# fpthink/EPC-Net

Measured on AMD Instinct MI355X. Metric: point-clouds/sec (4096 pts) descriptor extraction, higher is better.
Workload: dtype f16x3; 1 GPU; epc-net inference, batch 64x4096x3 fp32 per GPU, NetVLAD K=64, 256-D output (BASELINE.json configs[1]); num_points=4096, precision=EPC_PRECISION_F32 (include/epcnet.h), weights=seeded random init of the architecture (no checkpoint payloads exist), parallelism=independent clouds sharded over 1 GPU(s), no data-path collective

## Files before the change

### epc-net_amd/csrc/knn.hip

```cpp
#include "train_common.h"
#include <stdlib.h>

#define KNN_THREADS 1024
#define KNN_TILE 1024
#define KNN_CT 32
#define KNN_WAVES (KNN_THREADS / 64)
#define KNN_LDS_MAX_N 8192

__device__ __forceinline__ int fkey(float v) {
    const int b = __float_as_int(v);
    return b ^ ((b >> 31) & 0x7fffffff);
}
__device__ __forceinline__ float fkey_inv(int k) { return __int_as_float(k ^ ((k >> 31) & 0x7fffffff)); }

template <int KSEL>
__device__ __forceinline__ void topk_insert(float (&top)[KSEL], float v) {
#pragma unroll
    for (int s = 0; s < KSEL; ++s) {
        const float hi = fmaxf(top[s], v);
        v = fminf(top[s], v);
        top[s] = hi;
    }
}

__device__ __forceinline__ void topk_insert_key(int (&top)[20], int v) {
    int t;
    asm(
        "v_min_i32 %[t], %[k0], %[v]\n\tv_max_i32 %[k0], %[k0], %[v]\n\t"
        "v_min_i32 %[v], %[k1], %[t]\n\tv_max_i32 %[k1], %[k1], %[t]\n\t"
        "v_min_i32 %[t], %[k2], %[v]\n\tv_max_i32 %[k2], %[k2], %[v]\n\t"
        "v_min_i32 %[v], %[k3], %[t]\n\tv_max_i32 %[k3], %[k3], %[t]\n\t"
        "v_min_i32 %[t], %[k4], %[v]\n\tv_max_i32 %[k4], %[k4], %[v]\n\t"
        "v_min_i32 %[v], %[k5], %[t]\n\tv_max_i32 %[k5], %[k5], %[t]\n\t"
        "v_min_i32 %[t], %[k6], %[v]\n\tv_max_i32 %[k6], %[k6], %[v]\n\t"
        "v_min_i32 %[v], %[k7], %[t]\n\tv_max_i32 %[k7], %[k7], %[t]\n\t"
        "v_min_i32 %[t], %[k8], %[v]\n\tv_max_i32 %[k8], %[k8], %[v]\n\t"
        "v_min_i32 %[v], %[k9], %[t]\n\tv_max_i32 %[k9], %[k9], %[t]\n\t"
        "v_min_i32 %[t], %[k10], %[v]\n\tv_max_i32 %[k10], %[k10], %[v]\n\t"
        "v_min_i32 %[v], %[k11], %[t]\n\tv_max_i32 %[k11], %[k11], %[t]\n\t"
        "v_min_i32 %[t], %[k12], %[v]\n\tv_max_i32 %[k12], %[k12], %[v]\n\t"
        "v_min_i32 %[v], %[k13], %[t]\n\tv_max_i32 %[k13], %[k13], %[t]\n\t"
        "v_min_i32 %[t], %[k14], %[v]\n\tv_max_i32 %[k14], %[k14], %[v]\n\t"
        "v_min_i32 %[v], %[k15], %[t]\n\tv_max_i32 %[k15], %[k15], %[t]\n\t"
        "v_min_i32 %[t], %[k16], %[v]\n\tv_max_i32 %[k16], %[k16], %[v]\n\t"
        "v_min_i32 %[v], %[k17], %[t]\n\tv_max_i32 %[k17], %[k17], %[t]\n\t"
        "v_min_i32 %[t], %[k18], %[v]\n\tv_max_i32 %[k18], %[k18], %[v]\n\t"
        "v_min_i32 %[v], %[k19], %[t]\n\tv_max_i32 %[k19], %[k19], %[t]\n\t"
        : [v] "+v"(v), [t] "=&v"(t), [k0] "+v"(top[0]), [k1] "+v"(top[1]), [k2] "+v"(top[2]), [k3] "+v"(top[3]), [k4] "+v"(top[4]), [k5] "+v"(top[5]), [k6] "+v"(top[6]), [k7] "+v"(top[7]), [k8] "+v"(top[8]), [k9] "+v"(top[9]), [k10] "+v"(top[10]), [k11] "+v"(top[11]), [k12] "+v"(top[12]), [k13] "+v"(top[13]), [k14] "+v"(top[14]), [k15] "+v"(top[15]), [k16] "+v"(top[16]), [k17] "+v"(top[17]), [k18] "+v"(top[18]), [k19] "+v"(top[19]));
}

__device__ __forceinline__ void topk_insert_dist(float (&top)[20], float v) {
    asm(
        "v_med3_f32 %[k19], %[k18], %[k19], %[v]\n\t"
        "v_med3_f32 %[k18], %[k17], %[k18], %[v]\n\t"
        "v_med3_f32 %[k17], %[k16], %[k17], %[v]\n\t"
        "v_med3_f32 %[k16], %[k15], %[k16], %[v]\n\t"
        "v_med3_f32 %[k15], %[k14], %[k15], %[v]\n\t"
        "v_med3_f32 %[k14], %[k13], %[k14], %[v]\n\t"
        "v_med3_f32 %[k13], %[k12], %[k13], %[v]\n\t"
        "v_med3_f32 %[k12], %[k11], %[k12], %[v]\n\t"
        "v_med3_f32 %[k11], %[k10], %[k11], %[v]\n\t"
        "v_med3_f32 %[k10], %[k9], %[k10], %[v]\n\t"
        "v_med3_f32 %[k9], %[k8], %[k9], %[v]\n\t"
        "v_med3_f32 %[k8], %[k7], %[k8], %[v]\n\t"
        "v_med3_f32 %[k7], %[k6], %[k7], %[v]\n\t"
        "v_med3_f32 %[k6], %[k5], %[k6], %[v]\n\t"
        "v_med3_f32 %[k5], %[k4], %[k5], %[v]\n\t"
        "v_med3_f32 %[k4], %[k3], %[k4], %[v]\n\t"
        "v_med3_f32 %[k3], %[k2], %[k3], %[v]\n\t"
        "v_med3_f32 %[k2], %[k1], %[k2], %[v]\n\t"
        "v_med3_f32 %[k1], %[k0], %[k1], %[v]\n\t"
        "v_min_f32 %[k0], %[k0], %[v]\n\t"
        : [k0] "+v"(top[0]), [k1] "+v"(top[1]), [k2] "+v"(top[2]), [k3] "+v"(top[3]), [k4] "+v"(top[4]), [k5] "+v"(top[5]), [k6] "+v"(top[6]), [k7] "+v"(top[7]), [k8] "+v"(top[8]), [k9] "+v"(top[9]), [k10] "+v"(top[10]), [k11] "+v"(top[11]), [k12] "+v"(top[12]), [k13] "+v"(top[13]), [k14] "+v"(top[14]), [k15] "+v"(top[15]), [k16] "+v"(top[16]), [k17] "+v"(top[17]), [k18] "+v"(top[18]), [k19] "+v"(top[19])
        : [v] "v"(v));
}

__device__ __forceinline__ bool wave_any(bool p) { return __builtin_amdgcn_ballot_w64(p) != 0ull; }

#define KNN_BATCH 8
#define KNN_MASK_WORDS (KNN_LDS_MAX_N / KNN_BATCH / 32)
static_assert(32 % (KNN_CT / KNN_BATCH) == 0, "a tile's batch bits must not straddle a mask word");

template <int KSEL, bool CONV1, int BATCH>
__global__ __launch_bounds__(KNN_THREADS, BATCH == 4 ? 8 : 1) void knn_topk_culled_kernel(const float* __restrict__ xyz, int n, int cap,
                                                                      int32_t* __restrict__ idx,
                                                                      int32_t* __restrict__ cnt,
                                                                      float* __restrict__ kth_out,
                                                                      const float* __restrict__ conv1_pack,
                                                                      float* __restrict__ x32,
                                                                      unsigned short* __restrict__ x16, int idx_u16,
                                                                      int32_t* __restrict__ status) {
    extern __shared__ __attribute__((aligned(16))) float4 cand[];
    const int ntiles = (n + KNN_CT - 1) / KNN_CT;
    const int npad = ntiles * KNN_CT;
    float4* bb = cand + npad;
    float* s_margin = reinterpret_cast<float*>(bb + 2 * ntiles);
    constexpr int BPT = KNN_CT / BATCH;
    constexpr int MASKW = KNN_LDS_MAX_N / BATCH / 32;
    static_assert(32 % BPT == 0, "a tile's batch bits must not straddle a mask word");
    unsigned int* hitmask = reinterpret_cast<unsigned int*>(s_margin + 4) + (threadIdx.x >> 6) * MASKW;
    const int cloud = blockIdx.y;
    const int tid = threadIdx.x, lane = tid & 63, wave = __builtin_amdgcn_readfirstlane(tid >> 6);
    const float* pc = xyz + (size_t)cloud * n * 3;

    bool bad = false;
    for (int j = tid; j < npad; j += KNN_THREADS) {
        float4 v = make_float4(0.f, 0.f, 0.f, INFINITY);
        if (j < n) {
            v.x = pc[3 * j + 0];
            v.y = pc[3 * j + 1];
            v.z = pc[3 * j + 2];
            v.w = sq3(v.x, v.y, v.z);
            bad |= !(v.w <= 3.4028234664e38f);
        }
        cand[j] = v;
    }
    if (status && blockIdx.x == 0 && wave_any(bad) && lane == 0) atomicOr(status + cloud, EPC_STATUS_NONFINITE_INPUT);
    __syncthreads();
    if constexpr (CONV1) {
        const int q = tid & 15;
        const float4 w0 = *reinterpret_cast<const float4*>(conv1_pack + 4 * q);
        const float4 w1 = *reinterpret_cast<const float4*>(conv1_pack + 64 + 4 * q);
        const float4 w2 = *reinterpret_cast<const float4*>(conv1_pack + 128 + 4 * q);
        const float4 b = *reinterpret_cast<const float4*>(conv1_pack + 192 + 4 * q);
        const int p0 = blockIdx.x * KNN_THREADS;
        const int np = min(KNN_THREADS, n - p0);
        bool ovf = false;
        for (int t = tid; t < np * 16; t += KNN_THREADS) {
            const int g = p0 + (t >> 4);
            const float4 pt = cand[g];
            const float4 y = conv1_quad(pt.x, pt.y, pt.z, w0, w1, w2, b);
            const size_t row = (size_t)cloud * n + g;
            if (x32) *reinterpret_cast<float4*>(x32 + row * 64 + 4 * q) = y;
            if (x16) {
                reinterpret_cast<uint2*>(x16)[row * 16 + q] = pack_half4(y);
                ovf |= fmaxf(fmaxf(y.x, y.y), fmaxf(y.z, y.w)) > 65504.0f;
            }
        }
        if (status && x16 && wave_any(ovf) && lane == 0) atomicOr(status + cloud, EPC_STATUS_FP16_RANGE);
    }
    for (int t = wave * (64 / KNN_CT) + lane / KNN_CT; t < ntiles; t += KNN_WAVES * (64 / KNN_CT)) {
        const float4 v = cand[t * KNN_CT + (lane % KNN_CT)];
        const bool ok = v.w != INFINITY;
        float lx = ok ? v.x : INFINITY, ly = ok ? v.y : INFINITY, lz = ok ? v.z : INFINITY;
        float hx = ok ? v.x : -INFINITY, hy = ok ? v.y : -INFINITY, hz = ok ? v.z : -INFINITY;
#pragma unroll
        for (int off = KNN_CT / 2; off >= 1; off >>= 1) {
            lx = fminf(lx, __shfl_xor(lx, off));
            ly = fminf(ly, __shfl_xor(ly, off));
            lz = fminf(lz, __shfl_xor(lz, off));
            hx = fmaxf(hx, __shfl_xor(hx, off));
            hy = fmaxf(hy, __shfl_xor(hy, off));
            hz = fmaxf(hz, __shfl_xor(hz, off));
        }
        if ((lane % KNN_CT) == 0) {
            bb[2 * t] = make_float4(lx, ly, lz, 0.f);
            bb[2 * t + 1] = make_float4(hx, hy, hz, 0.f);
        }
    }
    __syncthreads();
    if (wave == 0) {
        float m = 0.f;
        for (int t = lane; t < ntiles; t += 64) {
            const float4 lo = bb[2 * t], hi = bb[2 * t + 1];
            const float ax = fmaxf(fabsf(lo.x), fabsf(hi.x)), ay = fmaxf(fabsf(lo.y), fabsf(hi.y)),
                        az = fmaxf(fabsf(lo.z), fabsf(hi.z));
            m = fmaxf(m, ax * ax + ay * ay + az * az);
        }
#pragma unroll
        for (int off = 32; off >= 1; off >>= 1) m = fmaxf(m, __shfl_xor(m, off));
        if (lane == 0) *s_margin = m * (256.0f * 5.9604645e-08f);
    }
    __syncthreads();
    const float margin = *s_margin;
    for (int o = lane; o < MASKW; o += 64) hitmask[o] = 0u;

    const int i = blockIdx.x * KNN_THREADS + tid;
    const bool valid = i < n;
    float xi = 0.f, yi = 0.f, zi = 0.f, sqi = 0.f;
    if (valid) {
        const float4 me = cand[i];
        xi = me.x;
        yi = me.y;
        zi = me.z;
        sqi = me.w;
    }
    static_assert(KSEL == 20, "topk_insert_key is written for the 20-slot list");
    float top[KSEL];
#pragma unroll
    for (int s = 0; s < KSEL; ++s) top[s] = valid ? INFINITY : -INFINITY;

    auto lower_bound = [&](int c) {
        const float4 lo = bb[2 * c], hi = bb[2 * c + 1];
        const float dx = fmaxf(fmaxf(lo.x - xi, xi - hi.x), 0.f);
        const float dy = fmaxf(fmaxf(lo.y - yi, yi - hi.y), 0.f);
        const float dz = fmaxf(fmaxf(lo.z - zi, zi - hi.z), 0.f);
        return dx * dx + dy * dy + dz * dz - margin;
    };
    auto pos_sq_dist = [&](const float4& q) {
#pragma clang fp contract(off)
        const float inner = (xi * q.x + yi * q.y) + zi * q.z;
        return __builtin_fmaf(-2.0f, inner, sqi) + q.w;
    };
#define thr top[KSEL - 1]
    auto scan1 = [&](int c) {
        if (!wave_any(lower_bound(c) <= thr)) return;
        const float4* tp = cand + c * KNN_CT;
#pragma unroll
        for (int k0 = 0; k0 < KNN_CT; k0 += BATCH) {
            float4 q[BATCH];
#pragma unroll
            for (int u = 0; u < BATCH; ++u) q[u] = tp[k0 + u];
            float d[BATCH];
#pragma unroll
            for (int u = 0; u < BATCH; ++u) d[u] = pos_sq_dist(q[u]);
            bool hit;
            if constexpr (BATCH == 8) {
                float dmin;
                asm("v_min3_f32 %0, %1, %2, %3\n\tv_min3_f32 %0, %0, %4, %5\n\tv_min3_f32 %0, %0, %6, %7\n\tv_min_f32 %0, %0, %8"
                    : "=&v"(dmin)
                    : "v"(d[0]), "v"(d[1]), "v"(d[2]), "v"(d[3]), "v"(d[4]), "v"(d[5]), "v"(d[6]), "v"(d[7]));
                hit = dmin <= thr;
            } else if constexpr (BATCH == 4) {
                float dmin;
                asm("v_min3_f32 %0, %1, %2, %3\n\tv_min_f32 %0, %0, %4" : "=&v"(dmin) : "v"(d[0]), "v"(d[1]), "v"(d[2]), "v"(d[3]));
                hit = dmin <= thr;
            } else {
                hit = false;
#pragma unroll
                for (int u = 0; u < BATCH; ++u) hit |= d[u] <= thr;
            }
            if (wave_any(hit)) {
                if (lane == 0) {
                    const int bit = c * BPT + k0 / BATCH;
                    hitmask[bit >> 5] |= 1u << (bit & 31);
                }
#pragma unroll
                for (int u = 0; u < BATCH; ++u) {
                    if (wave_any(d[u] < top[KSEL - 1])) {
                        topk_insert_dist(top, d[u]);
                    }
                }
            }
        }
    };

    const int t0 = (blockIdx.x * KNN_THREADS + wave * 64) / KNN_CT;
    constexpr int OWN = 64 / KNN_CT;
#pragma unroll
    for (int o = 0; o < OWN; ++o)
        if (t0 + o < ntiles) scan1(t0 + o);
    for (int d = 1; d < ntiles; ++d) {
        const int cl = t0 - d, cr = t0 + OWN - 1 + d;
        if (cl >= 0 && cl < ntiles) scan1(cl);
        if (cr < ntiles) scan1(cr);
    }
#undef thr
    const float kth = 0.0f - top[KSEL - 1];

    unsigned int count = 0;
    char* lists = reinterpret_cast<char*>(idx) + (size_t)cloud * n * cap * (idx_u16 ? 2 : 4);
    const float dk = -kth;
    const unsigned int ucap = (unsigned int)cap;
    auto pass2 = [&](auto wide) {
        constexpr int ESZ = decltype(wide)::value ? 4 : 2;
        const unsigned int row = (unsigned int)(valid ? i : 0) * ucap * ESZ;
        for (int c = 0; c < ntiles; ++c) {
            const int bit0 = c * BPT;
            const unsigned int bits = (hitmask[bit0 >> 5] >> (bit0 & 31)) & ((1u << BPT) - 1u);
            if (bits == 0u) continue;
            const float4* tp = cand + c * KNN_CT;
#pragma unroll
            for (int k0 = 0; k0 < KNN_CT; k0 += BATCH) {
                if (!((bits >> (k0 / BATCH)) & 1u)) continue;
                float4 q[BATCH];
#pragma unroll
                for (int u = 0; u < BATCH; ++u) q[u] = tp[k0 + u];
                float d[BATCH];
                bool hit = false;
#pragma unroll
                for (int u = 0; u < BATCH; ++u) {
                    d[u] = pos_sq_dist(q[u]);
                    hit |= d[u] <= dk;
                }
                if (wave_any(hit)) {
#pragma unroll
                    for (int u = 0; u < BATCH; ++u)
                        if (d[u] <= dk) {
                            if (valid && count < ucap) {
                                char* slot = lists + (row + count * ESZ);
                                if (ESZ == 4)
                                    *reinterpret_cast<int32_t*>(slot) = c * KNN_CT + k0 + u;
                                else
                                    *reinterpret_cast<unsigned short*>(slot) = (unsigned short)(c * KNN_CT + k0 + u);
                            }
                            ++count;
                        }
                }
            }
        }
    };
    if (idx_u16)
        pass2(std::false_type{});
    else
        pass2(std::true_type{});
    if (valid && count < (unsigned int)KSEL) {
        const size_t row = ((size_t)cloud * n + i) * cap;
        for (unsigned int c = count; c < (unsigned int)KSEL; ++c) {
            if (idx_u16)
                reinterpret_cast<unsigned short*>(idx)[row + c] = (unsigned short)i;
            else
                idx[row + c] = i;
        }
    }
    if (valid) {
        cnt[(size_t)cloud * n + i] = (int32_t)count;
        kth_out[(size_t)cloud * n + i] = kth;
    }
}

#define KQ_LANES 4

__device__ __forceinline__ float quad_max(float v) {
    float r;
    asm volatile("s_nop 1\n\t"
        "v_max_f32_dpp %0, %1, %1 quad_perm:[1,0,3,2] row_mask:0xf bank_mask:0xf\n\t"
        "s_nop 1\n\t"
        "v_max_f32_dpp %0, %0, %0 quad_perm:[2,3,0,1] row_mask:0xf bank_mask:0xf"
        : "=&v"(r)
        : "v"(v));
    return r;
}
template <int STEP>
__device__ __forceinline__ float dpp_quad_swap(float v) {
    float r;
    if (STEP == 0)
        asm volatile("s_nop 1\n\tv_mov_b32_dpp %0, %1 quad_perm:[1,0,3,2] row_mask:0xf bank_mask:0xf" : "=v"(r) : "v"(v));
    else
        asm volatile("s_nop 1\n\tv_mov_b32_dpp %0, %1 quad_perm:[2,3,0,1] row_mask:0xf bank_mask:0xf" : "=v"(r) : "v"(v));
    return r;
}

template <int KSEL, bool CONV1, int HMW>
__global__ __launch_bounds__(KNN_THREADS, 8) void knn_topk_quad_kernel(const float* __restrict__ xyz, int n, int cap,
                                                                       int32_t* __restrict__ idx, int32_t* __restrict__ cnt,
                                                                       float* __restrict__ kth_out,
                                                                       const float* __restrict__ conv1_pack,
                                                                       float* __restrict__ x32, unsigned short* __restrict__ x16,
                                                                       int idx_u16, int32_t* __restrict__ status, int rounds) {
    static_assert(KNN_CT == 32 && KSEL == 20, "written for 32-point tiles and the 20-slot list");
    extern __shared__ __attribute__((aligned(16))) float4 cand[];
    const int ntiles = (n + KNN_CT - 1) / KNN_CT;
    const int npad = ntiles * KNN_CT;
    float4* bb = cand + npad;
    float* s_margin = reinterpret_cast<float*>(bb + 2 * ntiles);
    static_assert(HMW * 32 * KNN_CT <= KNN_LDS_MAX_N, "mask words beyond the largest cloud");
    const int cloud = blockIdx.y;
    const int tid = threadIdx.x, lane = tid & 63, wave = __builtin_amdgcn_readfirstlane(tid >> 6), sub = lane & 3;
    const int nthreads = blockDim.x, nwaves = nthreads >> 6;
    const int wg_queries = nwaves * 16 * rounds;
    const float* pc = xyz + (size_t)cloud * n * 3;

    bool bad = false;
    for (int j = tid; j < npad; j += nthreads) {
        float4 v = make_float4(0.f, 0.f, 0.f, INFINITY);
        if (j < n) {
            v.x = pc[3 * j + 0];
            v.y = pc[3 * j + 1];
            v.z = pc[3 * j + 2];
            v.w = sq3(v.x, v.y, v.z);
            bad |= !(v.w <= 3.4028234664e38f);
        }
        cand[j] = v;
    }
    if (status && blockIdx.x == 0 && wave_any(bad) && lane == 0) atomicOr(status + cloud, EPC_STATUS_NONFINITE_INPUT);
    __syncthreads();
    if constexpr (CONV1) {
        const int q = tid & 15;
        const float4 w0 = *reinterpret_cast<const float4*>(conv1_pack + 4 * q);
        const float4 w1 = *reinterpret_cast<const float4*>(conv1_pack + 64 + 4 * q);
        const float4 w2 = *reinterpret_cast<const float4*>(conv1_pack + 128 + 4 * q);
        const float4 b = *reinterpret_cast<const float4*>(conv1_pack + 192 + 4 * q);
        const int p0 = blockIdx.x * wg_queries;
        const int np = min(wg_queries, n - p0);
        bool ovf = false;
        for (int t = tid; t < np * 16; t += nthreads) {
            const int g = p0 + (t >> 4);
            const float4 pt = cand[g];
            const float4 y = conv1_quad(pt.x, pt.y, pt.z, w0, w1, w2, b);
            const size_t row = (size_t)cloud * n + g;
            if (x32) *reinterpret_cast<float4*>(x32 + row * 64 + 4 * q) = y;
            if (x16) {
                reinterpret_cast<uint2*>(x16)[row * 16 + q] = pack_half4(y);
                ovf |= fmaxf(fmaxf(y.x, y.y), fmaxf(y.z, y.w)) > 65504.0f;
            }
        }
        if (status && x16 && wave_any(ovf) && lane == 0) atomicOr(status + cloud, EPC_STATUS_FP16_RANGE);
    }
    for (int t = wave * 2 + (lane >> 5); t < ntiles; t += nwaves * 2) {
        const float4 v = cand[t * KNN_CT + (lane & 31)];
        const bool ok = v.w != INFINITY;
        float lx = ok ? v.x : INFINITY, ly = ok ? v.y : INFINITY, lz = ok ? v.z : INFINITY;
        float hx = ok ? v.x : -INFINITY, hy = ok ? v.y : -INFINITY, hz = ok ? v.z : -INFINITY;
#pragma unroll
        for (int off = KNN_CT / 2; off >= 1; off >>= 1) {
            lx = fminf(lx, __shfl_xor(lx, off));
            ly = fminf(ly, __shfl_xor(ly, off));
            lz = fminf(lz, __shfl_xor(lz, off));
            hx = fmaxf(hx, __shfl_xor(hx, off));
            hy = fmaxf(hy, __shfl_xor(hy, off));
            hz = fmaxf(hz, __shfl_xor(hz, off));
        }
        if ((lane & 31) == 0) {
            bb[2 * t] = make_float4(lx, ly, lz, 0.f);
            bb[2 * t + 1] = make_float4(hx, hy, hz, 0.f);
        }
    }
    __syncthreads();
    const int nst = (ntiles + 3) >> 2;
    float4* sbb = reinterpret_cast<float4*>(s_margin + 4);
    for (int t = tid; t < nst; t += nthreads) {
        float4 lo = bb[8 * t], hi = bb[8 * t + 1];
        for (int r = 1; r < 4 && 4 * t + r < ntiles; ++r) {
            const float4 l = bb[8 * t + 2 * r], h = bb[8 * t + 2 * r + 1];
            lo.x = fminf(lo.x, l.x), lo.y = fminf(lo.y, l.y), lo.z = fminf(lo.z, l.z);
            hi.x = fmaxf(hi.x, h.x), hi.y = fmaxf(hi.y, h.y), hi.z = fmaxf(hi.z, h.z);
        }
        sbb[2 * t] = lo, sbb[2 * t + 1] = hi;
    }
    if (wave == 0) {
        float m = 0.f;
        for (int t = lane; t < ntiles; t += 64) {
            const float4 lo = bb[2 * t], hi = bb[2 * t + 1];
            const float ax = fmaxf(fabsf(lo.x), fabsf(hi.x)), ay = fmaxf(fabsf(lo.y), fabsf(hi.y)),
                        az = fmaxf(fabsf(lo.z), fabsf(hi.z));
            m = fmaxf(m, ax * ax + ay * ay + az * az);
        }
#pragma unroll
        for (int off = 32; off >= 1; off >>= 1) m = fmaxf(m, __shfl_xor(m, off));
        if (lane == 0) *s_margin = m * (256.0f * 5.9604645e-08f);
    }
    __syncthreads();
    const float margin = *s_margin;

    for (int round = 0; round < rounds; ++round) {
    const int i0 = blockIdx.x * wg_queries + (round * nwaves + wave) * 16;
    if (i0 >= n) break;
    const int i = i0 + (lane >> 2);
    const bool valid = i < n;
    unsigned long long hm[HMW];
#pragma unroll
    for (int w = 0; w < HMW; ++w) hm[w] = 0ull;
    float xi = 0.f, yi = 0.f, zi = 0.f, sqi = 0.f;
    if (valid) {
        const float4 me = cand[i];
        xi = me.x, yi = me.y, zi = me.z, sqi = me.w;
    }
    float top[KSEL];
#pragma unroll
    for (int s = 0; s < KSEL; ++s) top[s] = valid ? INFINITY : -INFINITY;

    auto lower_bound = [&](const float4* boxes, int c) {
        const float4 lo = boxes[2 * c], hi = boxes[2 * c + 1];
        const float dx = fmaxf(fmaxf(lo.x - xi, xi - hi.x), 0.f);
        const float dy = fmaxf(fmaxf(lo.y - yi, yi - hi.y), 0.f);
        const float dz = fmaxf(fmaxf(lo.z - zi, zi - hi.z), 0.f);
        return dx * dx + dy * dy + dz * dz - margin;
    };
    auto pos_sq_dist = [&](const float4& q) {
#pragma clang fp contract(off)
        const float inner = (xi * q.x + yi * q.y) + zi * q.z;
        return __builtin_fmaf(-2.0f, inner, sqi) + q.w;
    };
    auto thr_q = [&]() { return quad_max(top[4]); };
    auto scan1 = [&](int c) {
        const float4* tp = cand + c * KNN_CT + sub;
#pragma unroll
        for (int ub = 0; ub < 2; ++ub) {
            float4 q[4];
#pragma unroll
            for (int u = 0; u < 4; ++u) q[u] = tp[16 * ub + 4 * u];
            float d[4];
#pragma unroll
            for (int u = 0; u < 4; ++u) d[u] = pos_sq_dist(q[u]);
            float dmin;
            asm("v_min3_f32 %0, %1, %2, %3\n\tv_min_f32 %0, %0, %4" : "=&v"(dmin) : "v"(d[0]), "v"(d[1]), "v"(d[2]), "v"(d[3]));
            float thr = thr_q();
            if (wave_any(dmin <= thr)) {
                const int bit = c * 2 + ub;
                const unsigned long long bv = 1ull << (bit & 63);
#pragma unroll
                for (int w = 0; w < HMW; ++w) hm[w] |= (bit >> 6) == w ? bv : 0ull;
#pragma unroll
                for (int u = 0; u < 4; ++u) {
                    if (wave_any(d[u] < thr)) {
                        topk_insert_dist(top, d[u]);
                        thr = thr_q();
                    }
                }
            }
        }
    };

    const int t0 = i0 / KNN_CT;
    const int T0 = t0 >> 2;
    const int kmax = 2 * max(T0, nst - 1 - T0);
    auto super_of = [&](int k) { return T0 + ((k & 1) ? -((k + 1) >> 1) : (k >> 1)); };
    for (int kk = 0; kk <= kmax; kk += 4) {
        const int S = super_of(kk + sub);
        const bool in_s = S >= 0 && S < nst;
        const float lbs = in_s ? lower_bound(sbb, S) : INFINITY;
        const float thr_s = thr_q();
        const unsigned long long ms = __builtin_amdgcn_ballot_w64(in_s && lbs <= thr_s);
#pragma unroll 1
        for (int s = 0; s < 4; ++s) {
            if (!(ms & (0x1111111111111111ull << s))) continue;
            const int c0 = 4 * super_of(kk + s);
            const bool in = c0 + sub < ntiles;
            const float lb = in ? lower_bound(bb, c0 + sub) : INFINITY;
            const float thr = thr_q();
            const unsigned long long m = __builtin_amdgcn_ballot_w64(in && lb <= thr);
#pragma unroll
            for (int r = 0; r < 4; ++r)
                if (m & (0x1111111111111111ull << r)) scan1(c0 + r);
        }
    }
    {
        float c[KSEL];
#pragma unroll
        for (int s = 0; s < KSEL; ++s) {
            const float o = dpp_quad_swap<0>(top[KSEL - 1 - s]);
            asm("v_min_f32 %0, %1, %2" : "=v"(c[s]) : "v"(top[s]), "v"(o));
        }
        constexpr unsigned char CE[40][2] = {
            {0, 16}, {1, 17}, {2, 18},  {3, 19},  {16, 8},  {17, 9},  {18, 10}, {19, 11}, {4, 12},  {5, 13},
            {6, 14}, {7, 15}, {16, 4},  {17, 5},  {18, 6},  {19, 7},  {8, 12},  {9, 13},  {10, 14}, {11, 15},
            {0, 2},  {1, 3},  {16, 18}, {17, 19}, {4, 6},   {5, 7},   {8, 10},  {9, 11},  {12, 14}, {13, 15},
            {0, 1},  {2, 3},  {16, 17}, {18, 19}, {4, 5},   {6, 7},   {8, 9},   {10, 11}, {12, 13}, {14, 15}};
#pragma unroll
        for (int e = 0; e < 40; ++e) {
            float lo, hi;
            asm("v_min_f32 %0, %2, %3\n\tv_max_f32 %1, %2, %3" : "=&v"(lo), "=&v"(hi) : "v"(c[CE[e][0]]), "v"(c[CE[e][1]]));
            c[CE[e][0]] = lo, c[CE[e][1]] = hi;
        }
        constexpr unsigned char ORDER[KSEL] = {0, 1, 2, 3, 16, 17, 18, 19, 4, 5, 6, 7, 8, 9, 10, 11, 12, 13, 14, 15};
#pragma unroll
        for (int s = 0; s < KSEL; ++s) top[s] = c[ORDER[s]];
    }
    float top20 = -INFINITY;
#pragma unroll
    for (int s = 0; s < KSEL; ++s) {
        const float o = dpp_quad_swap<1>(top[KSEL - 1 - s]);
        float m;
        asm("v_min_f32 %0, %1, %2" : "=v"(m) : "v"(top[s]), "v"(o));
        asm("v_max_f32 %0, %1, %2" : "=v"(top20) : "v"(top20), "v"(m));
    }
    const float kth = 0.0f - top20;

    unsigned int count = 0;
    char* lists = reinterpret_cast<char*>(idx) + (size_t)cloud * n * cap * (idx_u16 ? 2 : 4);
    const float dk = -kth;
    const unsigned int ucap = (unsigned int)cap;
    const unsigned int qshift = lane & ~3u, below = (1u << sub) - 1u;
    auto pass2 = [&](auto wide) {
        constexpr int ESZ = decltype(wide)::value ? 4 : 2;
        const unsigned int row = (unsigned int)(valid ? i : 0) * ucap * ESZ;
        const int words = (2 * ntiles + 63) >> 6;
        for (int w = 0; w < words; ++w) {
            unsigned long long flagged = hm[0];
#pragma unroll
            for (int v = 1; v < HMW; ++v) flagged = w == v ? hm[v] : flagged;
            while (flagged) {
                const int bit = __builtin_ctzll(flagged);
                flagged &= flagged - 1ull;
                const int c = (w * 64 + bit) >> 1, ub = bit & 1;
                const float4* tp = cand + c * KNN_CT + sub;
                float4 q[4];
#pragma unroll
                for (int u = 0; u < 4; ++u) q[u] = tp[16 * ub + 4 * u];
                float d[4];
                bool hit = false;
#pragma unroll
                for (int u = 0; u < 4; ++u) {
                    d[u] = pos_sq_dist(q[u]);
                    hit |= d[u] <= dk;
                }
                if (wave_any(hit)) {
#pragma unroll
                    for (int u = 0; u < 4; ++u) {
                        const bool h = d[u] <= dk;
                        const unsigned long long m = __builtin_amdgcn_ballot_w64(h);
                        if (m == 0ull) continue;
                        const unsigned int qb = (unsigned int)(m >> qshift) & 15u;
                        const unsigned int pos = count + __builtin_popcount(qb & below);
                        if (h && valid && pos < ucap) {
                            char* slot = lists + (row + pos * ESZ);
                            const int j = c * KNN_CT + 16 * ub + 4 * u + sub;
                            if (ESZ == 4)
                                *reinterpret_cast<int32_t*>(slot) = j;
                            else
                                *reinterpret_cast<unsigned short*>(slot) = (unsigned short)j;
                        }
                        count += __builtin_popcount(qb);
                    }
                }
            }
        }
    };
    if (idx_u16)
        pass2(std::false_type{});
    else
        pass2(std::true_type{});
    if (valid && sub == 0) {
        if (count < (unsigned int)KSEL) {
            const size_t row = ((size_t)cloud * n + i) * cap;
            for (unsigned int c = count; c < (unsigned int)KSEL; ++c) {
                if (idx_u16)
                    reinterpret_cast<unsigned short*>(idx)[row + c] = (unsigned short)i;
                else
                    idx[row + c] = i;
            }
        }
        cnt[(size_t)cloud * n + i] = (int32_t)count;
        kth_out[(size_t)cloud * n + i] = kth;
    }
    }
}

template <int KSEL>
__global__ __launch_bounds__(KNN_THREADS) void knn_topk_stream_kernel(const float* __restrict__ xyz, int n, int cap,
                                                                      int32_t* __restrict__ idx,
                                                                      int32_t* __restrict__ cnt,
                                                                      float* __restrict__ kth_out,
                                                                      int32_t* __restrict__ status) {
    __shared__ float4 tile[KNN_TILE];
    bool bad = false;
    const int cloud = blockIdx.y;
    const int i = blockIdx.x * KNN_THREADS + threadIdx.x;
    const bool valid = i < n;
    const float* pc = xyz + (size_t)cloud * n * 3;
    float xi = 0.f, yi = 0.f, zi = 0.f;
    if (valid) {
        xi = pc[3 * i + 0];
        yi = pc[3 * i + 1];
        zi = pc[3 * i + 2];
    }
    const float sqi = sq3(xi, yi, zi);
    float top[KSEL];
#pragma unroll
    for (int s = 0; s < KSEL; ++s) top[s] = -INFINITY;

    auto load_tile = [&](int t0) {
        __syncthreads();
        for (int c = threadIdx.x; c < KNN_TILE; c += KNN_THREADS) {
            const int j = t0 + c;
            float4 v = make_float4(0.f, 0.f, 0.f, INFINITY);
            if (j < n) {
                v.x = pc[3 * j + 0];
                v.y = pc[3 * j + 1];
                v.z = pc[3 * j + 2];
                v.w = sq3(v.x, v.y, v.z);
                bad |= !(v.w <= 3.4028234664e38f);
            }
            tile[c] = v;
        }
        __syncthreads();
    };

    for (int t0 = 0; t0 < n; t0 += KNN_TILE) {
        load_tile(t0);
        const int lim = min(KNN_TILE, n - t0);
#pragma unroll 4
        for (int c = 0; c < lim; ++c) {
            const float4 q = tile[c];
            const float v = neg_sq_dist(sqi, xi, yi, zi, q.x, q.y, q.z, q.w);
            if (v > top[KSEL - 1]) topk_insert<KSEL>(top, v);
        }
    }
    const float kth = top[KSEL - 1];
    int count = 0;
    int32_t* my = idx + ((size_t)cloud * n + (valid ? i : 0)) * cap;
    for (int t0 = 0; t0 < n; t0 += KNN_TILE) {
        load_tile(t0);
        const int lim = min(KNN_TILE, n - t0);
#pragma unroll 4
        for (int c = 0; c < lim; ++c) {
            const float4 q = tile[c];
            const float v = neg_sq_dist(sqi, xi, yi, zi, q.x, q.y, q.z, q.w);
            if (v >= kth) {
                if (valid && count < cap) my[count] = t0 + c;
                ++count;
            }
        }
    }
    if (status && blockIdx.x == 0 && wave_any(bad) && (threadIdx.x & 63) == 0) atomicOr(status + cloud, EPC_STATUS_NONFINITE_INPUT);
    if (valid)
        for (int c = count; c < KSEL; ++c) my[c] = i;
    if (valid) {
        cnt[(size_t)cloud * n + i] = count;
        kth_out[(size_t)cloud * n + i] = kth;
    }
}

__global__ __launch_bounds__(256) void knn_mask_kernel(const float* __restrict__ xyz,
                                                       const float* __restrict__ kth, int n,
                                                       float* __restrict__ mask) {
    const int cloud = blockIdx.z;
    const int i = blockIdx.y;
    const int j = blockIdx.x * 256 + threadIdx.x;
    if (j >= n) return;
    const float* pc = xyz + (size_t)cloud * n * 3;
    const float xi = pc[3 * i], yi = pc[3 * i + 1], zi = pc[3 * i + 2];
    const float xj = pc[3 * j], yj = pc[3 * j + 1], zj = pc[3 * j + 2];
    const float a = neg_sq_dist(sq3(xi, yi, zi), xi, yi, zi, xj, yj, zj, sq3(xj, yj, zj));
    mask[((size_t)cloud * n + i) * n + j] = (a >= kth[(size_t)cloud * n + i]) ? 1.0f : 0.0f;
}

static int launch_knn(const float* xyz, int num_clouds, int n, int cap, int32_t* idx, int32_t* cnt, float* kth,
                      const float* conv1_pack, float* x32, void* x16, int idx_u16, int32_t* status, void* stream,
                      const char* who, bool one_lane = false) {
    dim3 grid((n + KNN_THREADS - 1) / KNN_THREADS, num_clouds);
    if (n <= KNN_LDS_MAX_N) {
        const int ntiles = (n + KNN_CT - 1) / KNN_CT;
        const size_t lds_bytes = ((size_t)ntiles * KNN_CT + 2 * (size_t)ntiles + 2) * sizeof(float4) +
                                 (size_t)KNN_WAVES * (KNN_LDS_MAX_N / 4 / 32) * sizeof(unsigned int);
        const int num_cus = epc_device_cu_count();
        const bool wide_grid = (long)grid.x * grid.y >= 2L * num_cus;
#define EPC_KNN_LAUNCH(C1, B)                                                                                                   \
    do {                                                                                                                        \
        if (int rc_ = epc_set_dyn_lds(reinterpret_cast<const void*>(knn_topk_culled_kernel<EPC_KNN_SELECT, C1, B>), lds_bytes, who)) \
            return rc_;                                                                                                         \
        hipLaunchKernelGGL((knn_topk_culled_kernel<EPC_KNN_SELECT, C1, B>), grid, dim3(KNN_THREADS), lds_bytes,                \
                           (hipStream_t)stream, xyz, n, cap, idx, cnt, kth, C1 ? conv1_pack : nullptr, C1 ? x32 : nullptr,     \
                           C1 ? (unsigned short*)x16 : nullptr, C1 ? idx_u16 : 0, status);                                      \
    } while (0)
        const bool quad = !one_lane;
        if (quad) {
            const int groups = (n + 15) / 16;
            const long slots = 2L * num_cus;
            int per_wg = (int)(((long)groups * num_clouds + slots - 1) / slots);
            per_wg = min(max(per_wg, 4), groups);
            while (per_wg < groups && (long)((groups + per_wg - 1) / per_wg) * num_clouds > slots) ++per_wg;
            const int rounds = (per_wg + KNN_WAVES - 1) / KNN_WAVES;
            const int g = (per_wg + rounds - 1) / rounds;
            const int wgs = (groups + g * rounds - 1) / (g * rounds);
            const dim3 qgrid(wgs, num_clouds), qblock(64 * g);
#define EPC_KNN_QLAUNCH(C1, W)                                                                                                   \
    do {                                                                                                                        \
        if (int rc_ = epc_set_dyn_lds(reinterpret_cast<const void*>(knn_topk_quad_kernel<EPC_KNN_SELECT, C1, W>), lds_bytes, who)) \
            return rc_;                                                                                                         \
        hipLaunchKernelGGL((knn_topk_quad_kernel<EPC_KNN_SELECT, C1, W>), qgrid, qblock, lds_bytes,                             \
                           (hipStream_t)stream, xyz, n, cap, idx, cnt, kth, C1 ? conv1_pack : nullptr, C1 ? x32 : nullptr,     \
                           C1 ? (unsigned short*)x16 : nullptr, C1 ? idx_u16 : 0, status, rounds);                              \
    } while (0)
            const bool small = ntiles <= 128;
            if (conv1_pack) {
                if (small) EPC_KNN_QLAUNCH(true, 4);
                else EPC_KNN_QLAUNCH(true, 8);
            } else {
                if (small) EPC_KNN_QLAUNCH(false, 4);
                else EPC_KNN_QLAUNCH(false, 8);
            }
#undef EPC_KNN_QLAUNCH
        } else if (conv1_pack) {
            if (wide_grid) EPC_KNN_LAUNCH(true, 4);
            else EPC_KNN_LAUNCH(true, 8);
        } else {
            if (wide_grid) EPC_KNN_LAUNCH(false, 4);
            else EPC_KNN_LAUNCH(false, 8);
        }
#undef EPC_KNN_LAUNCH
    } else {
        hipLaunchKernelGGL(knn_topk_stream_kernel<EPC_KNN_SELECT>, grid, dim3(KNN_THREADS), 0, (hipStream_t)stream,
                           xyz, n, cap, idx, cnt, kth, status);
    }
    EPC_CHECK_LAUNCH();
    return EPC_OK;
}

extern "C" int epc_knn_topk(const float* xyz, int num_clouds, int n, int cap, int32_t* idx, int32_t* cnt,
                            float* kth, void* stream) {
    EPC_CHECK_ARG(xyz && idx && cnt && kth, "null pointer");
    EPC_CHECK_ARG(num_clouds >= 0 && num_clouds <= 65535 && n >= EPC_KNN_SELECT,
                  "need num_points >= 20 (tf.nn.top_k k=20)");
    EPC_CHECK_ARG(cap >= EPC_KNN_SELECT, "list capacity must be >= 20");
    if (num_clouds == 0) return EPC_OK;
    return launch_knn(xyz, num_clouds, n, cap, idx, cnt, kth, nullptr, nullptr, nullptr, 0, nullptr, stream, __func__);
}

static int knn_topk_conv1_impl(const float* xyz, int num_clouds, int n, int cap, void* idx, int idx_u16, int32_t* cnt, float* kth,
                               const void* packed_conv1, float* x, void* x16, int32_t* status, void* stream, bool one_lane);

extern "C" int epc_knn_topk_form(const float* xyz, int num_clouds, int n, int cap, int32_t* idx, int32_t* cnt, float* kth, int form,
                                 void* stream) {
    EPC_CHECK_ARG(xyz && idx && cnt && kth, "null pointer");
    EPC_CHECK_ARG(num_clouds >= 0 && num_clouds <= 65535 && n >= EPC_KNN_SELECT && cap >= EPC_KNN_SELECT && (form == 0 || form == 1),
                  "need num_points >= 20, capacity >= 20, form 0 or 1");
    if (num_clouds == 0) return EPC_OK;
    return launch_knn(xyz, num_clouds, n, cap, idx, cnt, kth, nullptr, nullptr, nullptr, 0, nullptr, stream, __func__, form == 0);
}

extern "C" int epc_knn_topk_conv1_form(const float* xyz, int num_clouds, int n, int cap, void* idx, int idx_u16, int32_t* cnt,
                                       float* kth, const void* packed_conv1, float* x, void* x16, int32_t* status, int form,
                                       void* stream) {
    EPC_CHECK_ARG(form == 0 || form == 1, "form 0 or 1");
    return knn_topk_conv1_impl(xyz, num_clouds, n, cap, idx, idx_u16, cnt, kth, packed_conv1, x, x16, status, stream, form == 0);
}

extern "C" int epc_knn_topk_conv1(const float* xyz, int num_clouds, int n, int cap, void* idx, int idx_u16, int32_t* cnt,
                                  float* kth, const void* packed_conv1, float* x, void* x16, int32_t* status,
                                  void* stream) {
    return knn_topk_conv1_impl(xyz, num_clouds, n, cap, idx, idx_u16, cnt, kth, packed_conv1, x, x16, status, stream, false);
}

static int knn_topk_conv1_impl(const float* xyz, int num_clouds, int n, int cap, void* idx, int idx_u16, int32_t* cnt, float* kth,
                               const void* packed_conv1, float* x, void* x16, int32_t* status, void* stream, bool one_lane) {
    EPC_CHECK_ARG(xyz && idx && cnt && kth && packed_conv1 && (x || x16), "null pointer");
    EPC_CHECK_ARG(!idx_u16 || (n <= 65535 && n <= KNN_LDS_MAX_N), "2-byte lists need num_points <= 8192 (the LDS kernel)");
    EPC_CHECK_ARG(num_clouds >= 0 && num_clouds <= 65535 && n >= EPC_KNN_SELECT,
                  "need num_points >= 20 (tf.nn.top_k k=20)");
    EPC_CHECK_ARG(cap >= EPC_KNN_SELECT, "list capacity must be >= 20");
    if (num_clouds == 0) return EPC_OK;
    if (n > KNN_LDS_MAX_N) {
        int rc = launch_knn(xyz, num_clouds, n, cap, (int32_t*)idx, cnt, kth, nullptr, nullptr, nullptr, 0, status, stream, __func__);
        if (rc != EPC_OK) return rc;
        return epc_conv1_launch(xyz, packed_conv1, num_clouds * n, x, x16, status, n, stream);
    }
    return launch_knn(xyz, num_clouds, n, cap, (int32_t*)idx, cnt, kth, (const float*)packed_conv1, x, x16, idx_u16, status,
                      stream, __func__, one_lane);
}

extern "C" int epc_knn_mask(const float* xyz, const float* kth, int num_clouds, int n, float* mask,
                            void* stream) {
    EPC_CHECK_ARG(xyz && kth && mask, "null pointer");
    EPC_CHECK_ARG(num_clouds >= 0 && num_clouds <= 65535 && n > 0 && n <= 65535, "bad shape");
    if (num_clouds == 0) return EPC_OK;
    dim3 grid((n + 255) / 256, n, num_clouds);
    hipLaunchKernelGGL(knn_mask_kernel, grid, dim3(256), 0, (hipStream_t)stream, xyz, kth, n, mask);
    EPC_CHECK_LAUNCH();
    return EPC_OK;
}
```

Baseline: 63130 clouds/s.

## Warm-start KNN top-k from home tile and fuse threshold update into insert

Before the tile traversal, each quad's top-20 list is seeded from the first 20 candidates of its home super-tile using a branch-free fill. This gives a finite pruning threshold from the start, and those half-tiles are skipped in the main scan but forced into the second pass. Insertion now runs as one asm block of med3 ops that also recomputes the quad-max threshold with DPP, so a separate reduction per insert is no longer needed. Out-of-range bounds use NaN so a single compare drives the ballots, and pass2 reuses its ballots. These changes add hand-written asm and bookkeeping for skipped tiles, which brings correctness risk in edge cases.

Result: faster. 63820 clouds/s (median of 6 runs) (+1.1%).

```diff
diff --git a/epc-net_amd/csrc/knn.hip b/epc-net_amd/csrc/knn.hip
--- a/epc-net_amd/csrc/knn.hip
+++ b/epc-net_amd/csrc/knn.hip
@@ -331,6 +331,47 @@
         : "v"(v));
     return r;
 }
+__device__ __forceinline__ void topk_insert_dist_thr(float (&top)[20], float v, float& thr) {
+    asm volatile(
+        "v_med3_f32 %[k19], %[k18], %[k19], %[v]\n\t"
+        "v_med3_f32 %[k18], %[k17], %[k18], %[v]\n\t"
+        "v_med3_f32 %[k17], %[k16], %[k17], %[v]\n\t"
+        "v_med3_f32 %[k16], %[k15], %[k16], %[v]\n\t"
+        "v_med3_f32 %[k15], %[k14], %[k15], %[v]\n\t"
+        "v_med3_f32 %[k14], %[k13], %[k14], %[v]\n\t"
+        "v_med3_f32 %[k13], %[k12], %[k13], %[v]\n\t"
+        "v_med3_f32 %[k12], %[k11], %[k12], %[v]\n\t"
+        "v_med3_f32 %[k11], %[k10], %[k11], %[v]\n\t"
+        "v_med3_f32 %[k10], %[k9], %[k10], %[v]\n\t"
+        "v_med3_f32 %[k9], %[k8], %[k9], %[v]\n\t"
+        "v_med3_f32 %[k8], %[k7], %[k8], %[v]\n\t"
+        "v_med3_f32 %[k7], %[k6], %[k7], %[v]\n\t"
+        "v_med3_f32 %[k6], %[k5], %[k6], %[v]\n\t"
+        "v_med3_f32 %[k5], %[k4], %[k5], %[v]\n\t"
+        "v_med3_f32 %[k4], %[k3], %[k4], %[v]\n\t"
+        "v_med3_f32 %[k3], %[k2], %[k3], %[v]\n\t"
+        "v_med3_f32 %[k2], %[k1], %[k2], %[v]\n\t"
+        "v_max_f32_dpp %[t], %[k4], %[k4] quad_perm:[1,0,3,2] row_mask:0xf bank_mask:0xf\n\t"
+        "v_med3_f32 %[k1], %[k0], %[k1], %[v]\n\t"
+        "v_min_f32 %[k0], %[k0], %[v]\n\t"
+        "v_max_f32_dpp %[t], %[t], %[t] quad_perm:[2,3,0,1] row_mask:0xf bank_mask:0xf\n\t"
+        : [t] "=&v"(thr), [k0] "+v"(top[0]), [k1] "+v"(top[1]), [k2] "+v"(top[2]), [k3] "+v"(top[3]), [k4] "+v"(top[4]), [k5] "+v"(top[5]), [k6] "+v"(top[6]), [k7] "+v"(top[7]), [k8] "+v"(top[8]), [k9] "+v"(top[9]), [k10] "+v"(top[10]), [k11] "+v"(top[11]), [k12] "+v"(top[12]), [k13] "+v"(top[13]), [k14] "+v"(top[14]), [k15] "+v"(top[15]), [k16] "+v"(top[16]), [k17] "+v"(top[17]), [k18] "+v"(top[18]), [k19] "+v"(top[19])
+        : [v] "v"(v));
+}
+
+__device__ __forceinline__ void topk_fill(float (&top)[20], int len, float v) {
+    if (len == 0) {
+        top[0] = v;
+        return;
+    }
+#pragma unroll
+    for (int s = 19; s >= 1; --s) {
+        if (s == len) asm("v_max_f32 %0, %1, %2" : "=v"(top[s]) : "v"(top[s - 1]), "v"(v));
+        if (s < len) asm("v_med3_f32 %0, %1, %2, %3" : "=v"(top[s]) : "v"(top[s - 1]), "v"(top[s]), "v"(v));
+    }
+    asm("v_min_f32 %0, %1, %2" : "=v"(top[0]) : "v"(top[0]), "v"(v));
+}
+
 template <int STEP>
 __device__ __forceinline__ float dpp_quad_swap(float v) {
     float r;
@@ -473,10 +514,13 @@
         return __builtin_fmaf(-2.0f, inner, sqi) + q.w;
     };
     auto thr_q = [&]() { return quad_max(top[4]); };
+    float thr = valid ? INFINITY : -INFINITY;
+    int cwarm = -4, cskip = -1;
     auto scan1 = [&](int c) {
         const float4* tp = cand + c * KNN_CT + sub;
 #pragma unroll
         for (int ub = 0; ub < 2; ++ub) {
+            if (ub == 0 && c == cskip) continue;
             float4 q[4];
 #pragma unroll
             for (int u = 0; u < 4; ++u) q[u] = tp[16 * ub + 4 * u];
@@ -485,7 +529,6 @@
             for (int u = 0; u < 4; ++u) d[u] = pos_sq_dist(q[u]);
             float dmin;
             asm("v_min3_f32 %0, %1, %2, %3\n\tv_min_f32 %0, %0, %4" : "=&v"(dmin) : "v"(d[0]), "v"(d[1]), "v"(d[2]), "v"(d[3]));
-            float thr = thr_q();
             if (wave_any(dmin <= thr)) {
                 const int bit = c * 2 + ub;
                 const unsigned long long bv = 1ull << (bit & 63);
@@ -493,10 +536,7 @@
                 for (int w = 0; w < HMW; ++w) hm[w] |= (bit >> 6) == w ? bv : 0ull;
 #pragma unroll
                 for (int u = 0; u < 4; ++u) {
-                    if (wave_any(d[u] < thr)) {
-                        topk_insert_dist(top, d[u]);
-                        thr = thr_q();
-                    }
+                    if (wave_any(d[u] < thr)) topk_insert_dist_thr(top, d[u], thr);
                 }
             }
         }
@@ -506,20 +546,34 @@
     const int T0 = t0 >> 2;
     const int kmax = 2 * max(T0, nst - 1 - T0);
     auto super_of = [&](int k) { return T0 + ((k & 1) ? -((k + 1) >> 1) : (k >> 1)); };
+    if (4 * T0 + 2 < ntiles) {
+        cwarm = 4 * T0, cskip = cwarm + 2;
+#pragma unroll
+        for (int f = 0; f < 5; ++f) {
+            const float4* tp = cand + (cwarm + (f >> 1)) * KNN_CT + 16 * (f & 1) + sub;
+            float4 q[4];
+#pragma unroll
+            for (int u = 0; u < 4; ++u) q[u] = tp[4 * u];
+#pragma unroll
+            for (int u = 0; u < 4; ++u) topk_fill(top, 4 * f + u, pos_sq_dist(q[u]));
+        }
+#pragma unroll
+        for (int s = 0; s < KSEL; ++s) top[s] = valid ? top[s] : -INFINITY;
+        thr = thr_q();
+    }
     for (int kk = 0; kk <= kmax; kk += 4) {
         const int S = super_of(kk + sub);
         const bool in_s = S >= 0 && S < nst;
-        const float lbs = in_s ? lower_bound(sbb, S) : INFINITY;
-        const float thr_s = thr_q();
-        const unsigned long long ms = __builtin_amdgcn_ballot_w64(in_s && lbs <= thr_s);
+        const float lbs = in_s ? lower_bound(sbb, S) : __builtin_nanf("");
+        const unsigned long long ms = __builtin_amdgcn_ballot_w64(lbs <= thr);
 #pragma unroll 1
         for (int s = 0; s < 4; ++s) {
             if (!(ms & (0x1111111111111111ull << s))) continue;
             const int c0 = 4 * super_of(kk + s);
             const bool in = c0 + sub < ntiles;
-            const float lb = in ? lower_bound(bb, c0 + sub) : INFINITY;
-            const float thr = thr_q();
-            const unsigned long long m = __builtin_amdgcn_ballot_w64(in && lb <= thr);
+            const float lb = in ? lower_bound(bb, c0 + sub) : __builtin_nanf("");
+            unsigned long long m = __builtin_amdgcn_ballot_w64(lb <= thr);
+            if (c0 == cwarm) m &= ~0x3333333333333333ull;
 #pragma unroll
             for (int r = 0; r < 4; ++r)
                 if (m & (0x1111111111111111ull << r)) scan1(c0 + r);
@@ -565,11 +619,13 @@
     auto pass2 = [&](auto wide) {
         constexpr int ESZ = decltype(wide)::value ? 4 : 2;
         const unsigned int row = (unsigned int)(valid ? i : 0) * ucap * ESZ;
+        const unsigned int lcap = valid ? ucap : 0u;
         const int words = (2 * ntiles + 63) >> 6;
         for (int w = 0; w < words; ++w) {
             unsigned long long flagged = hm[0];
 #pragma unroll
             for (int v = 1; v < HMW; ++v) flagged = w == v ? hm[v] : flagged;
+            if (w == (2 * cwarm) >> 6) flagged |= 0x1full << ((2 * cwarm) & 63);
             while (flagged) {
                 const int bit = __builtin_ctzll(flagged);
                 flagged &= flagged - 1ull;
@@ -579,21 +635,20 @@
 #pragma unroll
                 for (int u = 0; u < 4; ++u) q[u] = tp[16 * ub + 4 * u];
                 float d[4];
-                bool hit = false;
+                unsigned long long hmask[4];
 #pragma unroll
                 for (int u = 0; u < 4; ++u) {
                     d[u] = pos_sq_dist(q[u]);
-                    hit |= d[u] <= dk;
+                    hmask[u] = __builtin_amdgcn_ballot_w64(d[u] <= dk);
                 }
-                if (wave_any(hit)) {
+                if ((hmask[0] | hmask[1] | hmask[2] | hmask[3]) != 0ull) {
 #pragma unroll
                     for (int u = 0; u < 4; ++u) {
-                        const bool h = d[u] <= dk;
-                        const unsigned long long m = __builtin_amdgcn_ballot_w64(h);
+                        const unsigned long long m = hmask[u];
                         if (m == 0ull) continue;
                         const unsigned int qb = (unsigned int)(m >> qshift) & 15u;
                         const unsigned int pos = count + __builtin_popcount(qb & below);
-                        if (h && valid && pos < ucap) {
+                        if (d[u] <= dk && pos < lcap) {
                             char* slot = lists + (row + pos * ESZ);
                             const int j = c * KNN_CT + 16 * ub + 4 * u + sub;
                             if (ESZ == 4)
```
